# JoernZheng/parallel-data-compression-and-decompression

Hardware: AMD Instinct MI355X
Metric: compress+decompress GB/s (raw bytes / (deflate + inflate time)), .zwz bit-exact (higher is better)
Workload: dtype u8; 1 GPU; 10000 x 262144 B text-like files per GPU -> 50000 chunks of <=65535 B (BASELINE configs[2]); chunk_bytes=65535, max_batch_chunks=51200, parallelism=shard-per-gpu x1

## Files before the change

### parallel-data-compression-and-decompression_amd/csrc/inflate_core.h

```cpp
#pragma once
#include "zwz_common.h"

namespace zwz {

constexpr uint32_t kLitFastBits = 10, kDistFastBits = 8;
constexpr uint32_t kBatch = 64;

enum InflateStatus : uint32_t {
    kInfEnd = 0,
    kInfNeedInput = 1,
    kInfDataError = 2,
    kInfOverflow = 3,
    kInfRunning = 4,
    kInfPending = 5
};

struct InflateTables {
    uint16_t lit_fast[1u << kLitFastBits];
    uint16_t dist_fast[1u << kDistFastBits];
    uint16_t lit_count[16], dist_count[16];
    uint16_t lit_sym[288], dist_sym[32];
    uint16_t lit_walk[2], dist_walk[2];
};

// ... 69 lines not shown
            uint32_t rev = bit_reverse(code, l);
            uint16_t e = (uint16_t)((sorted[idx] << 4) | l);
            for (uint32_t j = rev; j < (1u << fast_bits); j += 1u << l) fast[j] = e;
        }
        code <<= 1;
    }
    return left > 0 ? 1 : 0;
}

constexpr uint32_t kPkLit = 0, kPkMatch = 1, kPkEob = 2, kPkNone = 3, kPkErr = 5, kPkLen = 7;
ZWZ_HD uint16_t pack_lit_entry(uint32_t e ) {
    if (e == 0) return (uint16_t)(kPkNone << 13);
    const uint32_t l = e & 15u, s = e >> 4;
    const uint32_t kind = s < 256u ? kPkLit : s == 256u ? kPkEob : s < 286u ? kPkLen : kPkErr;
    return (uint16_t)(kind << 13 | s << 4 | (l + (kind == kPkLen ? length_extra_bits(s - 257u) : 0u)));
}
ZWZ_HD uint16_t pack_dist_entry(uint32_t e) {
    if (e == 0) return (uint16_t)(kPkNone << 13);
    const uint32_t l = e & 15u, d = e >> 4;
    return (uint16_t)((d < 30u ? kPkMatch : kPkErr) << 13 | d << 5 | (l + (d < 30u ? dist_extra_bits(d) : 0u)));
}
ZWZ_HD uint32_t unpack_lit_entry(uint32_t e) {
    const uint32_t kind = e >> 13, s = (e >> 4) & 511u, skip = e & 15u;
    if (kind == kPkNone) return 0u;
    return s << 4 | (skip - (kind == kPkLen ? length_extra_bits(s - 257u) : 0u));
}
ZWZ_HD uint32_t unpack_dist_entry(uint32_t e) {
    const uint32_t kind = e >> 13, d = (e >> 5) & 31u, skip = e & 31u;
    if (kind == kPkNone) return 0u;
    return d << 4 | (skip - (kind == kPkMatch ? dist_extra_bits(d) : 0u));
}

template <uint32_t kFmt = 0>
ZWZ_HD int decode_symbol(BitReader& br, const uint16_t* fast, uint32_t fast_bits, const uint16_t* count,
                         const uint16_t* sorted) {
    if (br.bits < 15) br.refill();
    uint32_t e = fast[br.peek(fast_bits)];
    if (kFmt == 1u) e = unpack_lit_entry(e); else if (kFmt == 2u) e = unpack_dist_entry(e);
    uint32_t l = e & 15u;
    if (e != 0 && l <= br.bits) { br.drop(l); return (int)(e >> 4); }
    int code = 0, first = 0, index = 0;
    for (uint32_t len = 1; len <= 15; len++) {
        if (br.bits < len) {
            if (len == 1) return -1;
            for (uint32_t l = len; l <= 15; l++) if (count[l]) return -1;
            return -2;
        }
        code |= (int)((br.hold >> (len - 1)) & 1u);
        int c = count[len];
        if (code - c < first) { br.drop(len); return sorted[index + (code - first)]; }
        index += c; first += c; first <<= 1; code <<= 1;
    }
    return -2;
}

struct InflateState {
    BitReader br;
    uint32_t out_pos;
    uint32_t last;
    uint32_t status;
};

ZWZ_HD bool inflate_begin(InflateState& st, const uint8_t* in, uint32_t n, uint32_t ring_mask = 0xffffffffu) {
    st.br.init(in, n, ring_mask); st.out_pos = 0; st.last = 0; st.status = kInfRunning;
    uint32_t cmf, flg;
    if (!st.br.take(8, cmf) || !st.br.take(8, flg)) { st.status = kInfNeedInput; return false; }
    if (((cmf << 8) + flg) % 31u || (cmf & 15u) != 8u || (cmf >> 4) > 7u || (flg & 0x20u)) { st.status = kInfDataError; return false; }
    return true;
}

enum BlockKind : uint32_t { kBlkStored = 0, kBlkHuffman = 1, kBlkStop = 2 };

ZWZ_HD bool inflate_block_type(InflateState& st, uint32_t& type) {
    if (!st.br.take(1, st.last)) { st.status = kInfNeedInput; return false; }
    if (!st.br.take(2, type)) { st.status = kInfNeedInput; return false; }
    return true;
}

ZWZ_HD bool inflate_dyn_begin(InflateState& st, uint8_t* cl , uint32_t& nlen, uint32_t& ndist) {
    BitReader& br = st.br;
    uint32_t ncode, v;
    if (br.bits < 14) br.refill();
    if (br.bits < 14) { st.status = kInfNeedInput; return false; }
    br.take(5, nlen); br.take(5, ndist); br.take(4, ncode);
    nlen += 257; ndist += 1; ncode += 4;
    if (nlen > 286 || ndist > 30) { st.status = kInfDataError; return false; }
    for (uint32_t i = 0; i < 19; i++) cl[i] = 0;
    for (uint32_t i = 0; i < ncode; i++) {
        if (!br.take(3, v)) { st.status = kInfNeedInput; return false; }
        uint32_t o = i < 3 ? 16u + i : i == 3 ? 0u : (i & 1u) ? 8u - ((i - 3u) >> 1) : 8u + ((i - 4u) >> 1);
        cl[o] = (uint8_t)v;
    }
    return true;
}

ZWZ_HD bool inflate_dyn_lengths(InflateState& st, const InflateTables& t, uint8_t* lens, uint32_t nlen, uint32_t ndist) {
    BitReader& br = st.br;
    uint32_t have = 0;
    while (have < nlen + ndist) {
        BitReader save = br;
        int sym = decode_symbol(br, t.dist_fast, 7, t.dist_count, t.dist_sym);
        if (sym == -1) { st.status = kInfNeedInput; return false; }
        if (sym == -2) { st.status = kInfDataError; return false; }
        if (sym < 16) { lens[have++] = (uint8_t)sym; continue; }
        uint32_t prev = 0, rep, xb = sym == 16 ? 2u : sym == 17 ? 3u : 7u, xv;
        if (!br.take(xb, xv)) { br = save; st.status = kInfNeedInput; return false; }
// ... 108 lines not shown
```

### parallel-data-compression-and-decompression_amd/csrc/zwz_kernels.hip

```cpp
#include <hip/hip_runtime.h>

#include <cstdio>
#include <cstdlib>
#include <cstring>
#include <type_traits>

#include "huff_core.h"
#include "inflate_core.h"
#include "stream_core.h"
#include "split_core.h"
#include "lz_core.h"
#include "zwz_md5.h"
#include "zwz_kernels.h"
#include "zwz_device.h"

#ifndef ZWZ_MATCH_EXP
#define ZWZ_MATCH_EXP 0
#endif
#if ZWZ_MATCH_EXP & 16
#define ZWZ_MSTAMP(ph) do { const uint64_t now_ = __builtin_amdgcn_s_memtime(); acc_[(ph)] += (uint32_t)(now_ - stamp_); stamp_ = now_; } while (0)
#else
#define ZWZ_MSTAMP(ph) do { } while (0)
#endif

// ... 1505 lines not shown
        __syncthreads();
    }
    ZWZ_ESTAMP(6);
    if (!in_slots) {
        for (uint32_t i = tid; i < ((n_out + 3) >> 2); i += kThreads) gout[i] = s_out[i];
    } else {
        const uint32_t body = s_blk[0].body_pos, slot_bits = enc_slot_bits<kThreads / 64u, kOutW>(wpw, body, s_blk[0].body_bits), slot0 = (body + 63u) & ~31u;
        const uint32_t sym_end = body + (uint32_t)__builtin_amdgcn_readlane((int)pre_l, kThreads / 64u);
        const uint32_t eob_code = s_blk[0].eob_code, ad_pos = 8u * (s_total_bytes - 4u);
        uint32_t d_of[kThreads / 64u];
#pragma unroll
        for (uint32_t i = 0; i < kThreads / 64u; i++) d_of[i] = body + (uint32_t)__builtin_amdgcn_readlane((int)pre_l, i);
        auto piece = [](uint32_t pos, uint32_t val, uint32_t bit) -> uint32_t {
            const int d = (int)pos - (int)bit;
            return d >= 32 || d <= -32 ? 0u : d >= 0 ? val << d : val >> (-d);
        };
        for (uint32_t j = tid; j < ((n_out + 3) >> 2); j += kThreads) {
            const uint32_t bit = j << 5;
            uint32_t v = j < (slot0 >> 5) ? s_out[j] : 0u;
            v |= piece(sym_end, eob_code, bit);
            if (bit + 32u > ad_pos) v |= piece(ad_pos, adler_be(), bit);
            if (bit + 32u > body && bit < sym_end) {
                uint32_t w = 0;
#pragma unroll
                for (uint32_t i = 1; i < kThreads / 64u; i++) w += d_of[i] <= bit ? 1u : 0u;
                for (; w < kThreads / 64u; w++) {
                    const uint32_t d = body + s_msum[w];
                    if (d >= bit + 32u) break;
                    const int sft = (int)bit - (int)d, len = (int)s_wsum[w];
                    const int lo = sft < 0 ? -sft : 0, hi = len - sft < 32 ? len - sft : 32;
                    if (hi > lo) {
                        const uint32_t at = (uint32_t)((int)(slot0 + w * slot_bits) + sft), aw = at >> 5;
                        const uint32_t x = __builtin_amdgcn_alignbit(s_out[aw + 1u], s_out[aw], at & 31u);
                        const uint32_t mask = (hi >= 32 ? 0xffffffffu : (1u << hi) - 1u) & ~((1u << lo) - 1u);
                        v |= x & mask;
                    }
                }
            }
            gout[j] = v;
        }
    }
    __syncthreads();
    ZWZ_ESTAMP(7);
  }
#if ZWZ_ENC_EXP & 16
    if (tid == ((ZWZ_ENC_EXP & 32) ? 960u : 0u)) for (uint32_t ph = 0; ph < 8; ph++) atomicAdd(&g_enc_times[ph], (unsigned long long)(eacc_[ph] >> 8));
#endif
}

#ifndef ZWZ_INF_EXP
#define ZWZ_INF_EXP 0
#endif
#if ZWZ_INF_EXP & 16
__device__ unsigned long long g_inf_times[8];
#define ZWZ_ISTAMP(ph) do { const uint64_t now_ = __builtin_amdgcn_s_memtime(); iacc_[(ph)] += (uint32_t)(now_ - istamp_); istamp_ = now_; } while (0)
#else
#define ZWZ_ISTAMP(ph) do { } while (0)
#endif
#ifndef ZWZ_INF_WAVES
#define ZWZ_INF_WAVES 5
#endif
constexpr uint32_t kInflateWavesPerSimd = ZWZ_INF_WAVES;
#ifndef ZWZ_WIN_SLOTS
#define ZWZ_WIN_SLOTS 4
#endif
constexpr uint32_t kInfRing = 2048, kInfFill = 1024, kInfMirror = ((8u * ZWZ_WIN_SLOTS + 4u + 15u) / 16u) * 16u;
constexpr uint32_t kWinSlots = ZWZ_WIN_SLOTS;
#ifndef ZWZ_WIN_PARTS
#define ZWZ_WIN_PARTS 2
#endif
constexpr uint32_t kWinParts = ZWZ_WIN_PARTS;

constexpr uint32_t kOwnCap = 1024;

static __device__ __forceinline__ int wave_build_decode_table(const uint8_t* lens, uint32_t n , uint16_t* fast , uint32_t fast_bits,
                                                              uint16_t* count, uint16_t* sorted, uint32_t& max_len, uint16_t* walk0, uint32_t* scr ) {
    const uint32_t lane = lane_id();
    uint32_t* s_cnt = scr; uint32_t* s_pos = scr + 16; uint32_t* s_fc = scr + 32;
    uint32_t l[5];
#pragma unroll
    for (uint32_t r = 0; r < 5; r++) { const uint32_t i = lane + 64u * r; l[r] = i < n ? (uint32_t)lens[i] : 0u; }
    if (lane < 16u) s_cnt[lane] = 0;
    for (uint32_t x = lane; x < (1u << fast_bits) / 8u; x += 64u) reinterpret_cast<uint4*>(fast)[x] = make_uint4(0, 0, 0, 0);
    __builtin_amdgcn_fence(__ATOMIC_ACQ_REL, "wavefront");
#pragma unroll
    for (uint32_t r = 0; r < 5; r++) if (l[r]) atomicAdd(&s_cnt[l[r]], 1u);
    __builtin_amdgcn_fence(__ATOMIC_ACQ_REL, "wavefront");
    int left = 1;
    uint32_t first = 0, index = 0, off = 0, code = 0, my_off = 0, my_fc = 0, my_cnt = 0;
    max_len = 0;
    for (uint32_t len = 1; len < 16u; len++) {
        const uint32_t c = s_cnt[len];
        if (c) max_len = len;
        left = (left << 1) - (int)c;
        if (left < 0) return -1;
        if (len <= fast_bits) { index += c; first += c; first <<= 1; }
        if (lane == len) { my_off = off; my_fc = code; my_cnt = c; }
        off += c; code = (code + c) << 1;
    }
    if (lane < 16u) { s_pos[lane] = my_off; s_fc[lane] = my_fc | my_off << 16; count[lane] = (uint16_t)my_cnt; }
    if (walk0 && lane == 0) { walk0[0] = (uint16_t)first; walk0[1] = (uint16_t)index; }
    __builtin_amdgcn_fence(__ATOMIC_ACQ_REL, "wavefront");
#pragma unroll
    for (uint32_t r = 0; r < 5; r++) {
        if (l[r]) {
            const uint32_t i = lane + 64u * r, pos = atomicAdd(&s_pos[l[r]], 1u);
            sorted[pos] = (uint16_t)i;
            if (l[r] <= fast_bits) {
                const uint32_t w = s_fc[l[r]], cd = (w & 0xffffu) + (pos - (w >> 16));
                const uint16_t e = (uint16_t)((i << 4) | l[r]);
                for (uint32_t j = bit_reverse(cd, l[r]); j < (1u << fast_bits); j += 1u << l[r]) fast[j] = e;
            }
        }
    }
    __builtin_amdgcn_fence(__ATOMIC_ACQ_REL, "wavefront");
    return left > 0 ? 1 : 0;
}

static __device__ __forceinline__ uint32_t wave_dyn_lengths(const uint8_t* ring, uint32_t bp, uint32_t total_bits, const uint16_t* cl_fast ,
                                                            uint8_t* lens, uint32_t want ) {
    const uint32_t lane = lane_id();
    uint32_t have = 0, carry = 0xffffffffu;
    while (have < want) {
        const uint32_t a = bp + lane;
        const uint32_t byte = (a >> 3) & (kInfRing - 1u);
        const uint32_t* w = reinterpret_cast<const uint32_t*>(ring) + (byte >> 2);
        const uint32_t bits = __builtin_amdgcn_alignbyte(w[1], w[0], byte & 3u) >> (a & 7u);
        const uint32_t e = cl_fast[bits & 127u], l = e & 15u, sym = e >> 4;
        const uint32_t xb = sym < 16u ? 0u : sym == 16u ? 2u : sym == 17u ? 3u : 7u, nb = l + xb;
        const uint32_t xv = (bits >> l) & ((1u << xb) - 1u);
        const bool bad = e == 0u || (uint64_t)bp + lane + nb > total_bits;
        const uint32_t jr = lane + (nb ? nb : 1u);
        uint64_t M = 0; uint32_t at = 0;
        while (at < 64u) { M |= 1ull << at; at = (uint32_t)__builtin_amdgcn_readlane((int)jr, (int)at); }
        const bool mine = (M >> lane) & 1ull;
        if (__ballot(mine && bad)) return 0xffffffffu;
        const uint32_t rep = !mine ? 0u : sym < 16u ? 1u : sym == 18u ? 11u + xv : 3u + xv;
        const uint32_t incl = wave_scan_incl(rep), before = have + incl - rep;
        const uint64_t over = __ballot(mine && before + rep > want), in_hdr = __ballot(mine && before < want);
        if (over & in_hdr) return 0xffffffffu;
        const bool live = mine && before < want;
        const uint32_t def = live && sym != 16u ? lane + 1u : 0u;
        const uint32_t near = wave_scan_max_incl(def);
        const uint32_t dval = sym < 16u ? sym : 0u;
        const uint32_t pv = near ? (uint32_t)__shfl((int)dval, (int)(near - 1u)) : carry;
        const uint32_t val = sym == 16u ? pv : dval;
        if (__ballot(live && sym == 16u && pv == 0xffffffffu)) return 0xffffffffu;
        if (live) for (uint32_t k = 0; k < rep; k++) lens[before + k] = (uint8_t)val;
        const uint64_t lv = __ballot(live);
        const uint32_t last = 63u - (uint32_t)__builtin_clzll(lv);
        carry = (uint32_t)__builtin_amdgcn_readlane((int)val, (int)last);
        have = (uint32_t)__builtin_amdgcn_readlane((int)(before + rep), (int)last);
        bp += (uint32_t)__builtin_amdgcn_readlane((int)jr, (int)last);
    }
    return bp;
}

struct InflateWaveMem {
    InflateTables t;
    uint8_t lens[320];
    uint32_t batch[kBatch], pos[kBatch];
    uint32_t sym[kBatch + 1];
    __attribute__((aligned(16))) uint8_t ownb[kOwnCap];
    __attribute__((aligned(16))) uint8_t ring[kInfRing + kInfMirror];
};

template <bool kSerialHeader, bool kStream, uint32_t kSplit = 0>
__global__ __launch_bounds__(kInflateThreads, kInflateWavesPerSimd) void inflate_kernel(const uint8_t* __restrict__ in, const uint64_t* __restrict__ in_off,
                                                                  const uint32_t* __restrict__ in_len, uint32_t n,
                                                                  uint8_t* __restrict__ out, uint64_t out_stride,
                                                                  uint32_t* __restrict__ out_len, uint32_t* __restrict__ status,
                                                                  const uint4* __restrict__ order ,
                                                                  StreamParams sp) {
    __shared__ InflateWaveMem s_mem[kInflateThreads / 64];
    const uint32_t wave = threadIdx.x >> 6, lane = lane_id();
    const uint32_t slot = blockIdx.x * (kInflateThreads / 64) + wave;
    if (slot >= n) return;
    const uint4 oe = order ? order[slot] : make_uint4(0, 0, 0, slot);
    const uint32_t chunk = oe.w;
    InflateWaveMem& m = s_mem[wave];
    const uint8_t* src = in + (order ? ((uint64_t)oe.y << 32 | oe.x) : in_off[chunk]);
    uint8_t* dst;
    uint32_t cap = kChunk;
    uint32_t seg_body = 0, seg_start = 0, seg_base = 0, seg_stream = 0, seg_fin = kSegBad;
    if constexpr (kSplit != 0) {
        static_assert(kStream, "the split forms are stream forms");
        const uint4 sgv = sp.seg[chunk];
        const uint4 sg = make_uint4(__builtin_amdgcn_readfirstlane(sgv.x), __builtin_amdgcn_readfirstlane(sgv.y), __builtin_amdgcn_readfirstlane(sgv.z), __builtin_amdgcn_readfirstlane(sgv.w));
        seg_body = sg.x; seg_stream = sg.y;
        if constexpr (kSplit == 1) { dst = nullptr; cap = kSplitMeasureCap; seg_base = sg.w; }
        else { dst = out + sp.out_off[seg_stream] + (sg.z & ~15u); seg_start = sg.z & 15u; cap = seg_start + sg.w; }
    } else if constexpr (kStream) {
        const uint64_t cap64 = sp.out_cap[chunk];
        if (oe.z >= kStreamMaxIn || cap64 >= kStreamMaxOut) {
            if (lane == 0) { sp.out_len[chunk] = 0; status[chunk] = kStrTooLarge; sp.rec[chunk] = make_uint4(0, 0, 0, kStrTooLarge); }
            return;
        }
        dst = out + sp.out_off[chunk];
        cap = (uint32_t)cap64;
    } else {
        dst = out + (size_t)chunk * out_stride;
    }
    const uint32_t nin = order ? oe.z : in_len[chunk];
    const uint32_t nin16 = (nin + 15u) & ~15u;

    uint32_t fill_end = 0;
    auto top_up = [&](uint32_t pos) {
        pos = __builtin_amdgcn_readfirstlane(pos);
        if (fill_end + kInfRing < pos + kInfFill) fill_end = pos & ~(kInfFill - 1u);
        while (fill_end < pos + kInfFill && fill_end < nin16) {
            const uint32_t o = fill_end + lane * 16u;
            uint4 v = make_uint4(0, 0, 0, 0);
            if (o < nin16) v = *reinterpret_cast<const uint4*>(src + o);
            *reinterpret_cast<uint4*>(m.ring + (o & (kInfRing - 1u))) = v;
            if ((o & (kInfRing - 1u)) < kInfMirror) *reinterpret_cast<uint4*>(m.ring + kInfRing + (o & (kInfRing - 1u))) = v;
            fill_end += kInfFill;
        }
        __builtin_amdgcn_fence(__ATOMIC_ACQ_REL, "wavefront");
    };

    InflateState st;
#if ZWZ_INF_EXP & 16
    uint64_t istamp_ = __builtin_amdgcn_s_memtime();
    uint32_t iacc_[8] = {0, 0, 0, 0, 0, 0, 0, 0};
#endif
    top_up(0);
    uint32_t go = 0;
    uint32_t origin = 0;
    StreamRecord rec{0, 0, 0, kInfRunning};
    if constexpr (kSplit == 2) origin = seg_start;
    auto skip_zeros = [&](uint32_t q) -> uint32_t {
        q = __builtin_amdgcn_readfirstlane(q);
        while (q < nin) {
            const uint32_t base = q & ~15u, o = base + lane * 16u;
            uint32_t hit = 0xffffffffu;
            if (o < nin16) {
                const uint4 v = *reinterpret_cast<const uint4*>(src + o);
                const uint32_t w[4] = {v.x, v.y, v.z, v.w};
#pragma unroll
                for (uint32_t b = 16; b-- > 0;) {
                    const uint32_t at = o + b;
                    if (((w[b >> 2] >> (8u * (b & 3u))) & 255u) && at >= q && at < nin) hit = at;
                }
            }
            const uint64_t any = __ballot(hit != 0xffffffffu);
            if (any) return (uint32_t)__builtin_amdgcn_readlane((int)hit, (int)__builtin_ctzll(any));
            q = base + 64u * 16u;
        }
        return nin;
    };
    if constexpr (kSplit != 0) {
        if (lane == 0) { st.br.init(m.ring, nin, kInfRing - 1u); st.out_pos = seg_start; st.last = 0; st.status = kInfRunning; st.br.seek_bit(seg_body * 8u); }
        go = 1;
    } else if constexpr (kStream) {
        const uint32_t nz = sp.wrap == kWrapGzip ? skip_zeros(0) : nin;
        uint32_t body = 0, sst = kInfRunning;
        if (lane == 0) {
            sst = stream_begin(sp.wrap, src, nin, nz, &body);
            st.br.init(m.ring, nin, kInfRing - 1u); st.out_pos = 0; st.last = 0; st.status = sst;
        }
        body = __builtin_amdgcn_readfirstlane(body);
        go = __builtin_amdgcn_readfirstlane(sst) == kInfRunning;
        if (go) {
            top_up(body);
            if (lane == 0) st.br.seek_bit(body * 8u);
        }
    } else {
        if (lane == 0) go = inflate_begin(st, m.ring, nin, kInfRing - 1u) ? 1u : 0u;
        go = __builtin_amdgcn_readfirstlane(go);
    }
    uint32_t fenced = 0;
    while (go) {
        uint32_t kind = kBlkStop, soff = 0, slen = 0, opos = 0;
        top_up(st.br.bit_pos() >> 3);
        {
            uint32_t v = 0, ok = 0;
            if (lane == 0) { opos = st.out_pos; ok = inflate_block_type(st, v) ? 1u : 0u; }
// ... 37 lines not shown
                }
                if (good) {
                    const int dr = wave_build_decode_table(m.lens + nlen, ndist, m.t.dist_fast, kDistFastBits, m.t.dist_count, m.t.dist_sym, max_len, m.t.dist_walk, m.batch);
                    if (v == 2u) { if (lane == 0) good = inflate_table_ok(st, dr, max_len, false) ? 1u : 0u; good = __builtin_amdgcn_readfirstlane(good); }
                }
                kind = good ? kBlkHuffman : kBlkStop;
            }
        }
        kind = __builtin_amdgcn_readfirstlane(kind);
        if (kind == kBlkStop) break;
        if (kind == kBlkHuffman) {
            __builtin_amdgcn_fence(__ATOMIC_ACQ_REL, "wavefront");
            for (uint32_t x = lane; x < (1u << kLitFastBits); x += 64u) m.t.lit_fast[x] = pack_lit_entry(m.t.lit_fast[x]);
            for (uint32_t x = lane; x < (1u << kDistFastBits); x += 64u) m.t.dist_fast[x] = pack_dist_entry(m.t.dist_fast[x]);
            __builtin_amdgcn_fence(__ATOMIC_ACQ_REL, "wavefront");
        }
        if (kind == kBlkStored) {
            soff = __builtin_amdgcn_readfirstlane(soff); slen = __builtin_amdgcn_readfirstlane(slen);
            opos = __builtin_amdgcn_readfirstlane(opos);
            uint32_t room = cap - opos, cp = slen < room ? slen : room;
            if constexpr (kSplit != 1) {
                const uint32_t head = min(cp, (16u - (opos & 15u)) & 15u);
                if (lane < head) dst[opos + lane] = src[soff + lane];
                const uint32_t s0 = soff + head, d0 = opos + head, sh = s0 & 3u;
                const uint32_t* sw = reinterpret_cast<const uint32_t*>(src + (s0 & ~3u));
                uint32_t nvec = (cp - head) >> 4;
                while (nvec && (s0 & ~3u) + 16u * nvec + 4u > nin16) nvec--;
                for (uint32_t v = lane; v < nvec; v += 64) {
                    const uint32_t* q = sw + 4u * v;
                    const uint32_t w0 = q[0], w1 = q[1], w2 = q[2], w3 = q[3], w4 = q[4];
                    *reinterpret_cast<uint4*>(dst + d0 + 16u * v) = make_uint4(__builtin_amdgcn_alignbyte(w1, w0, sh), __builtin_amdgcn_alignbyte(w2, w1, sh),
                                                                                __builtin_amdgcn_alignbyte(w3, w2, sh), __builtin_amdgcn_alignbyte(w4, w3, sh));
                }
                for (uint32_t i = head + 16u * nvec + lane; i < cp; i += 64) dst[opos + i] = src[soff + i];
            }
            uint32_t stop = 0;
            if (lane == 0) {
                st.out_pos += cp;
                if (cp < slen) st.status = kInfOverflow;
                stop = st.status != kInfRunning;
            }
            if (__builtin_amdgcn_readfirstlane(stop)) break;
        } else {
            enum : uint32_t { kLit = 0, kMatch = 1, kEob = 2, kSlow = 3, kNeed = 4, kErr = 5 };
            static_assert(kLit == kPkLit && kMatch == kPkMatch && kEob == kPkEob && kSlow == kPkNone && kErr == kPkErr, "the packed entries carry this enum");
            uint32_t bp = 0, opos_u = 0;
            if (lane == 0) { bp = st.br.bit_pos(); opos_u = st.out_pos; }
            bp = __builtin_amdgcn_readfirstlane(bp); opos_u = __builtin_amdgcn_readfirstlane(opos_u);
            const uint32_t total_bits = nin * 8u;
            uint32_t block_done = 0, stop_status = kInfRunning;
            ZWZ_ISTAMP(0);
            while (!block_done) {
                top_up(bp >> 3);
                uint32_t nsym = 0;
                uint32_t at = 0;
                constexpr uint32_t kOrbitEnd = 0xffffu;
#pragma unroll 1
              for (uint32_t wb = 0; wb < 64u * kWinSlots * kWinParts; wb += 64u * kWinSlots) {
                uint32_t inf[kWinSlots];
                const uint32_t near_end_s = __builtin_amdgcn_readfirstlane((uint32_t)((uint64_t)bp + wb + 64u * kWinSlots + 64u > total_bits));
                const uint32_t a0 = bp + wb + lane;
                const uint32_t byte0 = (a0 >> 3) & (kInfRing - 1u);
                uint32_t wd[2u * kWinSlots + 1u];
                {
                    const uint32_t* w = reinterpret_cast<const uint32_t*>(m.ring) + (byte0 >> 2);
#pragma unroll
                    for (uint32_t i = 0; i < 2u * kWinSlots + 1u; i++) wd[i] = w[i];
                }
#pragma unroll
                for (uint32_t r = 0; r < kWinSlots; r++) {
                    const uint32_t lo = __builtin_amdgcn_alignbyte(wd[2u * r + 1u], wd[2u * r], byte0), hi = __builtin_amdgcn_alignbyte(wd[2u * r + 2u], wd[2u * r + 1u], byte0);
                    const uint64_t bits = (((uint64_t)hi << 32) | lo) >> (a0 & 7u);
                    const uint32_t e = m.t.lit_fast[(uint32_t)bits & ((1u << kLitFastBits) - 1u)];
                    const uint32_t skip = e & 15u;
                    const uint32_t de = m.t.dist_fast[(uint32_t)(bits >> skip) & ((1u << kDistFastBits) - 1u)];
                    const bool is_len = (e >> 13) == kPkLen;
                    uint32_t kind = is_len ? de >> 13 : e >> 13;
                    const uint32_t nb = skip + (is_len ? de & 31u : 0u);
                    if (near_end_s) {
                        const int32_t avail = (int32_t)total_bits - (int32_t)(a0 + r * 64u);
                        if (avail <= 0 || ((kind <= kEob || kind == kErr) && (int32_t)nb > avail)) kind = kNeed;
                    }
                    inf[r] = kind | (nb << 3);
                }
                ZWZ_ISTAMP(1);
                uint32_t jr[kWinSlots];
#pragma unroll
                for (uint32_t r = 0; r < kWinSlots; r++) {
                    const uint32_t nbits = inf[r] >> 3;
                    jr[r] = (((inf[r] & 7u) <= kMatch) & (nbits != 0u)) ? wb + r * 64u + lane + nbits : kOrbitEnd;
                }
                uint64_t M[kWinSlots];
#pragma unroll
                for (uint32_t r = 0; r < kWinSlots; r++) {
                    uint64_t mk = 0;
                    const uint32_t lim = wb + 64u * (r + 1u);
                    auto hop = [&] { asm volatile("s_bitset1_b64 %0, %1" : "+s"(mk) : "s"(at)); at = (uint32_t)__builtin_amdgcn_readlane((int)jr[r], (int)at); };
                    while (at < lim) {
                        hop();
                        if (at >= lim) break;
                        hop();
                        if (at >= lim) break;
                        hop();
                        if (at >= lim) break;
                        hop();
                    }
                    M[r] = mk;
                }
#pragma unroll
                for (uint32_t r = 0; r < kWinSlots; r++) {
                    const uint32_t rank = nsym + rank_in(M[r]);
                    if (((M[r] >> lane) & 1ull) && rank <= kBatch) m.sym[rank] = (wb + r * 64u + lane) | inf[r] << 10;
                    nsym += (uint32_t)__popcll(M[r]);
                }
                ZWZ_ISTAMP(2);
                if (at >= kOrbitEnd || nsym > kBatch) break;
              }
                __builtin_amdgcn_fence(__ATOMIC_ACQ_REL, "wavefront");
                uint32_t cur = 0, k = 0, stop = 0xffu, opos_new = opos_u;
                {
                    const uint32_t have = (uint32_t)(lane < nsym);
                    const uint32_t sy = m.sym[lane];
                    const uint32_t kd = (sy >> 10) & 7u, s_off = sy & 0x3ffu, s_nb = sy >> 13;
                    uint32_t v;
                    {
                        const uint32_t a = bp + s_off;
                        const uint32_t byte = (a >> 3) & (kInfRing - 1u);
                        const uint32_t* w = reinterpret_cast<const uint32_t*>(m.ring) + (byte >> 2);
                        const uint32_t lo = __builtin_amdgcn_alignbyte(w[1], w[0], byte & 3u), hi = __builtin_amdgcn_alignbyte(w[2], w[1], byte & 3u);
                        const uint64_t bits = (((uint64_t)hi << 32) | lo) >> (a & 7u);
                        const uint32_t e = m.t.lit_fast[(uint32_t)bits & ((1u << kLitFastBits) - 1u)];
                        const uint32_t s = (e >> 4) & 511u, skip = e & 15u;
                        const uint32_t c = (s - 257u) & 31u;
                        const uint32_t xb = length_extra_bits(c);
                        const uint32_t len = length_base(c) + 3u + ((uint32_t)(bits >> ((skip - xb) & 15u)) & ((1u << xb) - 1u));
                        const uint64_t rest = bits >> skip;
                        const uint32_t de = m.t.dist_fast[(uint32_t)rest & ((1u << kDistFastBits) - 1u)];
                        const uint32_t d = (de >> 5) & 31u, dxb = dist_extra_bits(d) & 15u;
                        const uint32_t dist = dist_base(d) + 1u + ((uint32_t)(rest >> (((de & 31u) - dxb) & 31u)) & ((1u << dxb) - 1u));
                        v = kd == kMatch ? (len << 16) | dist : kd == kLit ? s : 0u;
                    }
                    const uint32_t is_lit = have & (uint32_t)(kd == kLit), is_match = have & (uint32_t)(kd == kMatch), mlen = v >> 16;
                    const uint32_t ol = is_lit + is_match * mlen;
                    const uint32_t sc = wave_scan_incl(ol);
                    const uint32_t pos = opos_u + sc - ol;
                    uint32_t ends;
                    if constexpr (kStream)
                        ends = have & ((uint32_t)(kd >= kEob) | (is_lit & (uint32_t)(pos >= cap)) |
                                       (is_match & ((uint32_t)((v & 0xffffu) > pos - origin) | (uint32_t)(mlen > cap - pos))));
                    else
                        ends = have & ((uint32_t)(kd >= kEob) | (is_lit & (uint32_t)(pos >= kChunk)) |
                                       (is_match & ((uint32_t)((v & 0xffffu) > pos) | (uint32_t)(pos + mlen > kChunk))));
                    const uint64_t C = __ballot(ends != 0);
                    if (C) {
                        const uint32_t lc = (uint32_t)__builtin_ctzll(C);
                        const uint32_t c_kind = (uint32_t)__builtin_amdgcn_readlane((int)kd, (int)lc), c_val = (uint32_t)__builtin_amdgcn_readlane((int)v, (int)lc);
                        const uint32_t c_off = (uint32_t)__builtin_amdgcn_readlane((int)s_off, (int)lc), c_nb = (uint32_t)__builtin_amdgcn_readlane((int)s_nb, (int)lc);
                        opos_new = (uint32_t)__builtin_amdgcn_readlane((int)pos, (int)lc);
                        cur = c_off;
                        k = lc;
                        if (c_kind == kLit) { stop = kErr; stop_status = kInfOverflow; }
                        else if (c_kind == kMatch) { stop = kErr; stop_status = (c_val & 0xffffu) > opos_new - origin ? kInfDataError : kInfOverflow; }
                        else if (c_kind == kEob) { cur += c_nb; stop = kEob; }
                        else { stop = c_kind; if (c_kind == kNeed) stop_status = kInfNeedInput; else if (c_kind == kErr) stop_status = kInfDataError; }
                    } else if (nsym > kBatch) {
                        k = kBatch;
                        cur = m.sym[kBatch] & 0x3ffu;
                        opos_new = opos_u + (uint32_t)__builtin_amdgcn_readlane((int)sc, 63);
                    } else {
                        k = nsym;
                        cur = (uint32_t)__builtin_amdgcn_readlane((int)(s_off + s_nb), (int)(nsym - 1u));
                        opos_new = opos_u + (uint32_t)__builtin_amdgcn_readlane((int)sc, 63);
                    }
                    m.batch[lane] = v;
                    m.pos[lane] = lane < k ? pos : 0xffffffffu;
                }
                bp += cur;
                __builtin_amdgcn_fence(__ATOMIC_ACQ_REL, "wavefront");
                ZWZ_ISTAMP(3);
                const uint32_t bstart = opos_u;
                const uint32_t bbytes = opos_new - bstart;
                opos_u = opos_new;
                if constexpr (kSplit != 1) {
                const bool mapped = bbytes <= kOwnCap;
                if (mapped) {
                    for (uint32_t i = lane; i < (bbytes + 15u) >> 4; i += 64u) reinterpret_cast<uint4*>(m.ownb)[i] = make_uint4(0, 0, 0, 0);
                    __builtin_amdgcn_fence(__ATOMIC_ACQ_REL, "wavefront");
                    if (lane < k) m.ownb[m.pos[lane] - bstart] = (uint8_t)(lane + 1u);
                    __builtin_amdgcn_fence(__ATOMIC_ACQ_REL, "wavefront");
                    uint32_t carry = 0;
                    for (uint32_t j0 = 0; j0 < bbytes; j0 += 64) {
                        const uint32_t o = max(wave_scan_max_incl((uint32_t)m.ownb[j0 + lane]), carry);
                        m.ownb[j0 + lane] = (uint8_t)o;
                        carry = (uint32_t)__builtin_amdgcn_readlane((int)o, 63);
                    }
                    __builtin_amdgcn_fence(__ATOMIC_ACQ_REL, "wavefront");
                }
                ZWZ_ISTAMP(4);
                auto owner = [&](uint32_t pos, uint32_t& ov, uint32_t& op) {
                    uint32_t lo = 0;
                    if (mapped) lo = (uint32_t)m.ownb[pos - bstart] - 1u;
                    else {
#pragma unroll
                        for (uint32_t stp = 32; stp >= 1; stp >>= 1) { const uint32_t q = m.pos[(lo + stp) & 63u]; if (q <= pos) lo += stp; }
                    }
                    ov = m.batch[lo]; op = m.pos[lo];
                };
                auto source_of = [&](uint32_t at, uint32_t op, uint32_t d, bool live) -> uint32_t {
                    const uint32_t off = at - op;
                    uint32_t from = at - d;
                    if (__ballot(live && off >= d)) from = off < d ? from : op - d + off % (d | (uint32_t)!live);
                    return from;
                };
                bool need_fence = false;
                for (uint32_t j0 = 0; j0 < bbytes; j0 += 64) {
                    const uint32_t pos = bstart + j0 + lane;
                    const bool in = j0 + lane < bbytes;
                    uint32_t ov = 0, op = 0;
                    owner(in ? pos : bstart, ov, op);
                    bool lit = ov < 256u;
                    uint32_t src = source_of(pos, op, ov & 0xffffu, in && !lit);
                    while (__ballot(in && !lit && src >= bstart)) {
                        const bool go2 = in && !lit && src >= bstart;
                        uint32_t ov2 = 0, op2 = 0;
                        owner(go2 ? src : bstart, ov2, op2);
                        const uint32_t s2 = source_of(src, op2, ov2 & 0xffffu, go2 && ov2 >= 256u);
                        if (go2) {
                            if (ov2 < 256u) { lit = true; ov = ov2; }
                            else src = s2;
                        }
                    }
                    const uint64_t far = __ballot(in && !lit && src + 1u > fenced);
                    if (far && !(ZWZ_INF_EXP & 2)) { __builtin_amdgcn_fence(__ATOMIC_ACQ_REL, "workgroup"); __builtin_amdgcn_s_waitcnt(0); fenced = bstart; }
                    if (in) dst[pos] = lit ? (uint8_t)ov : __hip_atomic_load(&dst[src], __ATOMIC_RELAXED, __HIP_MEMORY_SCOPE_AGENT);
                    (void)need_fence;
                }
                }
                ZWZ_ISTAMP(5);
                if (stop == kEob) block_done = 1;
                else if (stop == kSlow) {
                    uint32_t k1 = 0, d1 = 0, nbp = bp, nop = opos_u, stt = kInfRunning;
                    if (lane == 0) {
                        st.br.seek_bit(bp); st.out_pos = opos_u;
                        bool d;
                        if constexpr (kStream) k1 = inflate_decode_batch<true, true>(st, m.t, cap, m.batch, m.pos, d, 1u, origin);
                        else k1 = inflate_decode_batch<true>(st, m.t, kChunk, m.batch, m.pos, d, 1u);
                        d1 = d; nbp = st.br.bit_pos(); nop = st.out_pos; stt = st.status;
                    }
                    k1 = __builtin_amdgcn_readfirstlane(k1); d1 = __builtin_amdgcn_readfirstlane(d1);
                    bp = __builtin_amdgcn_readfirstlane(nbp); opos_u = __builtin_amdgcn_readfirstlane(nop);
                    stt = __builtin_amdgcn_readfirstlane(stt);
                    __builtin_amdgcn_fence(__ATOMIC_ACQ_REL, "wavefront");
                    if constexpr (kSplit != 1) if (k1) {
                        const uint32_t mv = m.batch[0], mp = m.pos[0];
                        if (mv < 256u) { if (lane == 0) dst[mp] = (uint8_t)mv; }
                        else {
                            const uint32_t len = mv >> 16, dist = mv & 0xffffu;
                            const uint32_t from = mp - dist, span = len < dist ? len : dist;
                            if (from + span > fenced) {
                                __builtin_amdgcn_fence(__ATOMIC_ACQ_REL, "workgroup");
                                __builtin_amdgcn_s_waitcnt(0);
                                fenced = mp;
                            }
                            for (uint32_t i = lane; i < len; i += 64) dst[mp + i] = __hip_atomic_load(&dst[from + (i % dist)], __ATOMIC_RELAXED, __HIP_MEMORY_SCOPE_AGENT);
                        }
                    }
                    if (d1) { block_done = 1; stop_status = stt; }
                } else if (stop != 0xffu) { block_done = 1; }
            }
            uint32_t halt = 0;
            if (lane == 0) {
                st.out_pos = opos_u;
                if (stop_status != kInfRunning) st.status = stop_status;
                else st.br.seek_bit(bp);
                halt = st.status != kInfRunning;
            }
            if (__builtin_amdgcn_readfirstlane(halt)) break;
        }
        if constexpr (kSplit != 0) {
            uint32_t fin = kSegBad;
            if (lane == 0) fin = split_stop(st.last, kind == kBlkStored && slen == 0u);
            seg_fin = __builtin_amdgcn_readfirstlane(fin);
            if (seg_fin != kSegBad) break;
        } else if constexpr (kStream) {
            uint32_t more = 0, next = 0;
            if (lane == 0 && st.last) {
                const uint32_t q = (st.br.bit_pos() + 7u) >> 3;
                st.status = stream_trailer(sp.wrap, src, nin, q, st.out_pos, st.out_pos - origin, rec, &next);
                more = st.status == kInfRunning;
                if (!more) rec.status = st.status;
            }
            if (__builtin_amdgcn_readfirstlane(more)) {
                const uint32_t nz = skip_zeros(next);
                uint32_t body = 0, sst = kInfRunning;
                if (lane == 0) { sst = gzip_next_member(src, nin, nz, &body); st.status = sst; st.last = 0; }
                body = __builtin_amdgcn_readfirstlane(body);
                if (__builtin_amdgcn_readfirstlane(sst) != kInfRunning) break;
                origin = __builtin_amdgcn_readfirstlane(st.out_pos);
                top_up(body);
                if (lane == 0) st.br.seek_bit(body * 8u);
                continue;
            }
            if (__builtin_amdgcn_readfirstlane((uint32_t)(st.status != kInfRunning))) break;
        } else {
            uint32_t fin = 0;
            if (lane == 0 && st.last) { st.status = kInfEnd; fin = 1; }
            if (__builtin_amdgcn_readfirstlane(fin)) break;
        }
    }
    if constexpr (kSplit == 1) {
        if (lane == 0) sp.meas[chunk] = make_uint4(seg_fin, seg_base + ((st.br.bit_pos() + 7u) >> 3), st.out_pos, st.status);
    } else if constexpr (kSplit == 2) {
        if (lane == 0 && !(seg_fin != kSegBad && st.out_pos == cap)) sp.bad[seg_stream] = 1;
    } else if constexpr (kStream) {
        if (lane == 0) {
            sp.out_len[chunk] = st.out_pos; status[chunk] = st.status;
            sp.rec[chunk] = make_uint4(rec.checked, rec.expect, rec.has_check, st.status);
        }
    } else {
        if (lane == 0) { out_len[chunk] = st.out_pos; status[chunk] = st.status; }
    }
#if ZWZ_INF_EXP & 16
    ZWZ_ISTAMP(6);
    if (lane == 0) for (uint32_t ph = 0; ph < 8; ph++) atomicAdd(&g_inf_times[ph], (unsigned long long)(iacc_[ph] >> 8));
#endif
}

#define ZWZ_TRY(x) do { hipError_t e_ = (x); if (e_ != hipSuccess) return e_; } while (0)

constexpr uint32_t kProbeRounds = 384;
__global__ __launch_bounds__(kLinksThreads) void exchange_order_probe_kernel(uint32_t* __restrict__ violations) {
    extern __shared__ __attribute__((aligned(16))) uint32_t tab[];
    constexpr uint32_t kBuckets = 32768u;
    uint32_t* area = tab + kBuckets + 4u;
    const uint32_t tid = threadIdx.x, lane = lane_id(), wave = tid >> 6;
    for (uint32_t i = tid; i < kBuckets; i += kLinksThreads) tab[i] = 0xdead0000u + i;
    for (uint32_t i = tid; i < 4096u; i += kLinksThreads) area[i] = i;
    __syncthreads();
    if (wave != 0) {
        uint4* a4 = reinterpret_cast<uint4*>(area) + (wave - 1u) * 128u + lane;
        uint4 v = a4[0];
        for (uint32_t it = 0; it < 3u * kProbeRounds; it++) {
            a4[64 * (it & 1u)] = make_uint4(v.x + it, v.y ^ it, v.z + lane, v.w);
            v = a4[64 * ((it + 1u) & 1u)];
        }
        if (v.x == 0xffffffffu && v.y == 0x12345678u) violations[1] = v.z;
        return;
    }
    typedef __attribute__((address_space(3))) uint32_t* lds_word_ptr;
    const uint32_t tab_a = (uint32_t)(uintptr_t)(lds_word_ptr)tab;
    uint32_t bad = 0, rng = 0x9e3779b9u * (lane + 1u) + 0x85ebca6bu * (blockIdx.x + 1u);
    for (uint32_t r = 0; r < kProbeRounds; r++) {
        rng = rng * 1664525u + 1013904223u;
        const uint32_t spread = 1u << (3u * (r % 6u));
        const uint32_t base = (0x9e3779b1u * (r + 17u * blockIdx.x)) & (kBuckets - 1u) & ~(spread - 1u);
        const uint32_t a = base + ((rng >> 11) & (spread - 1u));
        const uint32_t la = tab_a + 4u * a, mine = 0x10000u * (r + 1u) + lane;
        uint32_t pre, old, post;
        asm volatile("ds_read_b32 %0, %3\n\ts_waitcnt lgkmcnt(0)\n\t"
                     "ds_wrxchg_rtn_b32 %1, %3, %4\n\ts_waitcnt lgkmcnt(0)\n\t"
                     "ds_read_b32 %2, %3\n\ts_waitcnt lgkmcnt(0)"
                     : "=&v"(pre), "=&v"(old), "=&v"(post) : "v"(la), "v"(mine) : "memory");
        uint32_t want = pre, last = lane;
        for (uint32_t j = 0; j < 64; j++) {
            const uint32_t aj = (uint32_t)__builtin_amdgcn_readlane((int)a, (int)j);
            if (aj != a) continue;
            if (j < lane) want = 0x10000u * (r + 1u) + j;
            if (j > lane) last = j;
        }
        bad += (uint32_t)(old != want) + (uint32_t)(post != 0x10000u * (r + 1u) + last);
    }
    if (bad) atomicAdd(violations, bad);
}

hipError_t probe_exchange_order(hipStream_t s, bool* holds) {
    uint32_t* d = nullptr;
    uint32_t h[2] = {1, 0};
// ... 212 lines not shown
    };
    auto grouped_add = [&](uint32_t c, bool live) -> uint32_t {
        uint32_t slot = 0;
        uint64_t todo = __builtin_amdgcn_ballot_w64(live);
        if (todo) {
            const uint32_t c0 = (uint32_t)__builtin_amdgcn_readlane((int)c, (int)__builtin_ctzll(todo));
            const uint64_t m = __builtin_amdgcn_ballot_w64(live && c == c0);
            if (__popcll(todo & ~m) > 8) {
                if (live) slot = atomicAdd(&s_bin[c], 1u);
                return slot;
            }
        }
        while (todo) {
            const uint32_t c0 = (uint32_t)__builtin_amdgcn_readlane((int)c, (int)__builtin_ctzll(todo));
            const uint64_t m = __builtin_amdgcn_ballot_w64(live && c == c0);
            uint32_t base = 0;
            if (lane_id() == (uint32_t)__builtin_ctzll(m)) base = atomicAdd(&s_bin[c0], (uint32_t)__popcll(m));
            base = (uint32_t)__builtin_amdgcn_readlane((int)base, (int)__builtin_ctzll(m));
            if (live && c == c0) slot = base + rank_in(m);
            todo &= ~m;
        }
        return slot;
    };
    for (uint32_t i = tid; i - tid < n; i += 1024u) (void)grouped_add(i < n ? cls(in_len(i)) : 0u, i < n);
    __syncthreads();
    const bool keep = __syncthreads_count(tid < 256u && s_bin[tid] != 0u) <= 2;
    if (keep) {
        for (uint32_t i = tid; i < n; i += 1024u) { const uint64_t off = in_off[i]; order[i] = make_uint4((uint32_t)off, (uint32_t)(off >> 32), in_len(i), i); }
        return;
    }
    if (tid < 64u) {
        const uint32_t a = s_bin[4 * tid], b = s_bin[4 * tid + 1], c = s_bin[4 * tid + 2], d = s_bin[4 * tid + 3];
        const uint32_t own = a + b + c + d, ex = wave_scan_incl(own) - own;
        s_bin[4 * tid] = ex; s_bin[4 * tid + 1] = ex + a; s_bin[4 * tid + 2] = ex + a + b; s_bin[4 * tid + 3] = ex + a + b + c;
    }
    __syncthreads();
    for (uint32_t i = tid; i - tid < n; i += 1024u) {
        const uint32_t len = i < n ? in_len(i) : 0u;
        const uint32_t slot = grouped_add(cls(len), i < n);
        if (i < n) { const uint64_t off = in_off[i]; order[slot] = make_uint4((uint32_t)off, (uint32_t)(off >> 32), len, i); }
    }
}

hipError_t launch_inflate(const InflateArgs& a, hipStream_t s) {
    if (a.n == 0) return hipSuccess;
    const uint32_t per = kInflateThreads / 64;
    if (a.order) hipLaunchKernelGGL(inflate_order_kernel<uint32_t>, dim3(1), dim3(1024), 0, s, a.in_off, a.in_len, a.n, a.order);
    if (a.serial_header) hipLaunchKernelGGL((inflate_kernel<true, false>), dim3((a.n + per - 1) / per), dim3(kInflateThreads), 0, s, a.in, a.in_off, a.in_len, a.n, a.out,
                                            a.out_stride, a.out_len, a.status, (const uint4*)a.order, StreamParams{});
    else hipLaunchKernelGGL((inflate_kernel<false, false>), dim3((a.n + per - 1) / per), dim3(kInflateThreads), 0, s, a.in, a.in_off, a.in_len, a.n, a.out,
                            a.out_stride, a.out_len, a.status, (const uint4*)a.order, StreamParams{});
#if ZWZ_INF_EXP & 16
    if (getenv("ZWZ_INF_TIMES")) {
        unsigned long long h[8], z[8] = {0};
        ZWZ_TRY(hipStreamSynchronize(s));
        ZWZ_TRY(hipMemcpyFromSymbol(h, HIP_SYMBOL(g_inf_times), sizeof h));
        ZWZ_TRY(hipMemcpyToSymbol(HIP_SYMBOL(g_inf_times), z, sizeof z));
        fprintf(stderr, "ZWZ_INF_TIMES n=%u header=%llu decode=%llu orbit=%llu symbols=%llu owners=%llu copy=%llu other=%llu\n", a.n, h[0], h[1], h[2], h[3], h[4], h[5], h[6]);
    }
#endif
    return hipGetLastError();
}

hipError_t launch_inflate_streams(const InflateStreamArgs& a, hipStream_t s) {
    if (a.n == 0) return hipSuccess;
    const uint32_t per = kInflateThreads / 64;
    hipLaunchKernelGGL(inflate_order_kernel<uint64_t>, dim3(1), dim3(1024), 0, s, a.in_off, a.in_len, a.n, a.order);
    const StreamParams sp{a.out_off, a.out_cap, a.out_len, a.rec, a.wrap};
    if (a.serial_header) hipLaunchKernelGGL((inflate_kernel<true, true>), dim3((a.n + per - 1) / per), dim3(kInflateThreads), 0, s, a.in, a.in_off, nullptr, a.n, a.out,
                                            0, nullptr, a.status, (const uint4*)a.order, sp);
    else hipLaunchKernelGGL((inflate_kernel<false, true>), dim3((a.n + per - 1) / per), dim3(kInflateThreads), 0, s, a.in, a.in_off, nullptr, a.n, a.out,
                            0, nullptr, a.status, (const uint4*)a.order, sp);
    return hipGetLastError();
}

hipError_t launch_inflate_split(const InflateSplitArgs& a, hipStream_t s) {
    if (a.n == 0) return hipSuccess;
    const uint32_t per = kInflateThreads / 64;
    hipLaunchKernelGGL(inflate_order_kernel<uint64_t>, dim3(1), dim3(1024), 0, s, a.seg_in_off, a.seg_in_len, a.n, a.order);
    StreamParams sp{};
    sp.out_off = a.out_off; sp.seg = a.seg; sp.meas = a.meas; sp.bad = a.bad;
    const dim3 grid((a.n + per - 1) / per), block(kInflateThreads);
#define ZWZ_SPLIT_LAUNCH(h, k) hipLaunchKernelGGL((inflate_kernel<h, true, k>), grid, block, 0, s, a.in, a.seg_in_off, nullptr, a.n, a.out, 0, nullptr, nullptr, (const uint4*)a.order, sp)
    if (a.measure) { if (a.serial_header) ZWZ_SPLIT_LAUNCH(true, 1); else ZWZ_SPLIT_LAUNCH(false, 1); }
    else { if (a.serial_header) ZWZ_SPLIT_LAUNCH(true, 2); else ZWZ_SPLIT_LAUNCH(false, 2); }
#undef ZWZ_SPLIT_LAUNCH
    return hipGetLastError();
}

}
```

Baseline: 22.12 GB/s.

## Resolve long Huffman codes in-wave instead of falling back to serial decode

When the orbit walk of the parallel inflate stops on a symbol whose code is longer than the fast table covers, the wave now decodes that long literal/length/distance cooperatively. Each lane probes one code length using canonical-code prefix scans. The decoded value is stored in a small side buffer, the symbol's entry is patched, and the orbit walk continues. This avoids dropping into the lane-0 sequential decode path and ending the batch early. It adds ballot/scan work per long code, a cap of eight such symbols per round, and extra registers and shared memory. Counters for rounds, sequential fallbacks and resolved symbols are added to the instrumentation.

```diff
diff --git a/parallel-data-compression-and-decompression_amd/csrc/inflate_core.h b/parallel-data-compression-and-decompression_amd/csrc/inflate_core.h
--- a/parallel-data-compression-and-decompression_amd/csrc/inflate_core.h
+++ b/parallel-data-compression-and-decompression_amd/csrc/inflate_core.h
@@ -145,6 +145,43 @@
         index += c; first += c; first <<= 1; code <<= 1;
     }
     return -2;
+}
+
+ZWZ_HD bool long_code_probe(uint32_t x, uint32_t l , uint32_t count_l, uint32_t before, uint32_t weight_before, uint32_t& idx) {
+    const uint32_t first = weight_before >> (15u - l);
+    const uint32_t d = bit_reverse(x & ((1u << l) - 1u), l) - first;
+    idx = before + d;
+    return d < count_l;
+}
+struct LongSymbol { uint32_t kind, nb, value; };
+template <class Pick>
+ZWZ_HD LongSymbol long_symbol(uint64_t bits, const InflateTables& t, Pick pick) {
+    const LongSymbol none{kPkNone, 0u, 0u};
+    const uint32_t e = t.lit_fast[(uint32_t)bits & ((1u << kLitFastBits) - 1u)];
+    uint32_t s = (e >> 4) & 511u, skip = e & 15u;
+    if ((e >> 13) == kPkNone) {
+        const uint32_t p = pick(t.lit_count, (uint32_t)bits & 0x7fffu);
+        if (!p) return none;
+        s = t.lit_sym[p >> 4];
+        if (s < 256u) return LongSymbol{kPkLit, p & 15u, s};
+        if (s == 256u || s >= 286u) return none;
+        skip = (p & 15u) + length_extra_bits(s - 257u);
+    } else if ((e >> 13) != kPkLen) return none;
+    const bool long_len = (e >> 13) == kPkNone;
+    const uint32_t c = s - 257u, xb = length_extra_bits(c);
+    const uint32_t len = c == 28u ? 258u : length_base(c) + 3u + ((uint32_t)(bits >> (skip - xb)) & ((1u << xb) - 1u));
+    const uint64_t rest = bits >> skip;
+    const uint32_t de = t.dist_fast[(uint32_t)rest & ((1u << kDistFastBits) - 1u)];
+    uint32_t d = (de >> 5) & 31u, dl = (de & 31u) - dist_extra_bits(d);
+    if ((de >> 13) == kPkNone) {
+        const uint32_t p = pick(t.dist_count, (uint32_t)rest & 0x7fffu);
+        if (!p) return none;
+        d = t.dist_sym[p >> 4]; dl = p & 15u;
+        if (d >= 30u) return none;
+    } else if ((de >> 13) != kPkMatch || !long_len) return none;
+    const uint32_t dxb = dist_extra_bits(d);
+    const uint32_t dist = dist_base(d) + 1u + ((uint32_t)(rest >> dl) & ((1u << dxb) - 1u));
+    return LongSymbol{kPkMatch, skip + dl + dxb, len << 16 | dist};
 }
 
 struct InflateState {
diff --git a/parallel-data-compression-and-decompression_amd/csrc/zwz_kernels.hip b/parallel-data-compression-and-decompression_amd/csrc/zwz_kernels.hip
--- a/parallel-data-compression-and-decompression_amd/csrc/zwz_kernels.hip
+++ b/parallel-data-compression-and-decompression_amd/csrc/zwz_kernels.hip
@@ -1581,10 +1581,12 @@
 #define ZWZ_INF_EXP 0
 #endif
 #if ZWZ_INF_EXP & 16
-__device__ unsigned long long g_inf_times[8];
+__device__ unsigned long long g_inf_times[8], g_inf_counts[4];
+#define ZWZ_ICOUNT(c) do { icnt_[(c)]++; } while (0)
 #define ZWZ_ISTAMP(ph) do { const uint64_t now_ = __builtin_amdgcn_s_memtime(); iacc_[(ph)] += (uint32_t)(now_ - istamp_); istamp_ = now_; } while (0)
 #else
 #define ZWZ_ISTAMP(ph) do { } while (0)
+#define ZWZ_ICOUNT(c) do { } while (0)
 #endif
 #ifndef ZWZ_INF_WAVES
 #define ZWZ_INF_WAVES 5
@@ -1600,6 +1602,7 @@
 #endif
 constexpr uint32_t kWinParts = ZWZ_WIN_PARTS;
 
+constexpr uint32_t kLongCap = 8;
 constexpr uint32_t kOwnCap = 1024;
 
 static __device__ __forceinline__ int wave_build_decode_table(const uint8_t* lens, uint32_t n , uint16_t* fast , uint32_t fast_bits,
@@ -1690,6 +1693,7 @@
     uint8_t lens[320];
     uint32_t batch[kBatch], pos[kBatch];
     uint32_t sym[kBatch + 1];
+    uint32_t side[kLongCap];
     __attribute__((aligned(16))) uint8_t ownb[kOwnCap];
     __attribute__((aligned(16))) uint8_t ring[kInfRing + kInfMirror];
 };
@@ -1751,7 +1755,7 @@
     InflateState st;
 #if ZWZ_INF_EXP & 16
     uint64_t istamp_ = __builtin_amdgcn_s_memtime();
-    uint32_t iacc_[8] = {0, 0, 0, 0, 0, 0, 0, 0};
+    uint32_t iacc_[8] = {0, 0, 0, 0, 0, 0, 0, 0}, icnt_[3] = {0, 0, 0};
 #endif
     top_up(0);
     uint32_t go = 0;
@@ -1895,7 +1899,9 @@
             ZWZ_ISTAMP(0);
             while (!block_done) {
                 top_up(bp >> 3);
+                ZWZ_ICOUNT(0);
                 uint32_t nsym = 0;
+                uint32_t nlong = 0;
                 uint32_t at = 0;
                 constexpr uint32_t kOrbitEnd = 0xffffu;
 #pragma unroll 1
@@ -1935,8 +1941,11 @@
                 }
                 uint64_t M[kWinSlots];
 #pragma unroll
+                for (uint32_t r = 0; r < kWinSlots; r++) M[r] = 0;
+              for (;;) {
+#pragma unroll
                 for (uint32_t r = 0; r < kWinSlots; r++) {
-                    uint64_t mk = 0;
+                    uint64_t mk = M[r];
                     const uint32_t lim = wb + 64u * (r + 1u);
                     auto hop = [&] { asm volatile("s_bitset1_b64 %0, %1" : "+s"(mk) : "s"(at)); at = (uint32_t)__builtin_amdgcn_readlane((int)jr[r], (int)at); };
                     while (at < lim) {
@@ -1950,6 +1959,35 @@
                     }
                     M[r] = mk;
                 }
+                if (__builtin_expect(at != kOrbitEnd || near_end_s || nlong >= kLongCap || (ZWZ_INF_EXP & 4), 1)) break;
+                uint32_t rs = 0, last = 0, li = kErr;
+#pragma unroll
+                for (uint32_t r = 0; r < kWinSlots; r++)
+                    if (M[r]) { rs = r; last = 63u - (uint32_t)__builtin_clzll(M[r]); li = (uint32_t)__builtin_amdgcn_readlane((int)inf[r], (int)last); }
+                if (__builtin_expect((li & 7u) != kSlow, 1)) break;
+                const uint32_t loff = wb + rs * 64u + last, a = bp + loff;
+                const uint32_t byte = (a >> 3) & (kInfRing - 1u);
+                const uint32_t* w = reinterpret_cast<const uint32_t*>(m.ring) + (byte >> 2);
+                const uint32_t lo = __builtin_amdgcn_alignbyte(w[1], w[0], byte & 3u), hi = __builtin_amdgcn_alignbyte(w[2], w[1], byte & 3u);
+                const LongSymbol ls = long_symbol((((uint64_t)hi << 32) | lo) >> (a & 7u), m.t, [&](const uint16_t* count, uint32_t x) -> uint32_t {
+                    const uint32_t l = lane & 15u, c = count[l], wt = c << (15u - l);
+                    uint32_t idx = 0;
+                    const bool hit = long_code_probe(x, l | (uint32_t)(l == 0u), c, wave_scan_incl(c) - c, wave_scan_incl(wt) - wt, idx) && lane - 1u < 15u;
+                    const uint64_t b = __ballot(hit);
+                    if (!b) return 0u;
+                    const uint32_t won = (uint32_t)__builtin_ctzll(b);
+                    return won | (uint32_t)__builtin_amdgcn_readlane((int)idx, (int)won) << 4;
+                });
+                if (__builtin_amdgcn_readfirstlane(ls.kind) == kPkNone) break;
+                const uint32_t l_nb = __builtin_amdgcn_readfirstlane(ls.nb);
+                const uint32_t patched = __builtin_amdgcn_readfirstlane(ls.kind) | l_nb << 3 | (nlong + 1u) << 9;
+#pragma unroll
+                for (uint32_t r = 0; r < kWinSlots; r++) if (rs == r && lane == last) inf[r] = patched;
+                if (lane == 0) m.side[nlong] = ls.value;
+                nlong++;
+                ZWZ_ICOUNT(2);
+                at = loff + l_nb;
+              }
 #pragma unroll
                 for (uint32_t r = 0; r < kWinSlots; r++) {
                     const uint32_t rank = nsym + rank_in(M[r]);
@@ -1964,7 +2002,7 @@
                 {
                     const uint32_t have = (uint32_t)(lane < nsym);
                     const uint32_t sy = m.sym[lane];
-                    const uint32_t kd = (sy >> 10) & 7u, s_off = sy & 0x3ffu, s_nb = sy >> 13;
+                    const uint32_t kd = (sy >> 10) & 7u, s_off = sy & 0x3ffu, s_nb = (sy >> 13) & 63u;
                     uint32_t v;
                     {
                         const uint32_t a = bp + s_off;
@@ -1983,6 +2021,7 @@
                         const uint32_t dist = dist_base(d) + 1u + ((uint32_t)(rest >> (((de & 31u) - dxb) & 31u)) & ((1u << dxb) - 1u));
                         v = kd == kMatch ? (len << 16) | dist : kd == kLit ? s : 0u;
                     }
+                    if (nlong) { const uint32_t sx = sy >> 19; if (have & (uint32_t)(sx != 0u)) v = m.side[(sx - 1u) & (kLongCap - 1u)]; }
                     const uint32_t is_lit = have & (uint32_t)(kd == kLit), is_match = have & (uint32_t)(kd == kMatch), mlen = v >> 16;
                     const uint32_t ol = is_lit + is_match * mlen;
                     const uint32_t sc = wave_scan_incl(ol);
@@ -2083,6 +2122,7 @@
                 if (stop == kEob) block_done = 1;
                 else if (stop == kSlow) {
                     uint32_t k1 = 0, d1 = 0, nbp = bp, nop = opos_u, stt = kInfRunning;
+                    ZWZ_ICOUNT(1);
                     if (lane == 0) {
                         st.br.seek_bit(bp); st.out_pos = opos_u;
                         bool d;
@@ -2166,6 +2206,7 @@
 #if ZWZ_INF_EXP & 16
     ZWZ_ISTAMP(6);
     if (lane == 0) for (uint32_t ph = 0; ph < 8; ph++) atomicAdd(&g_inf_times[ph], (unsigned long long)(iacc_[ph] >> 8));
+    if (lane == 0) for (uint32_t c = 0; c < 3; c++) atomicAdd(&g_inf_counts[c], (unsigned long long)icnt_[c]);
 #endif
 }
 
@@ -2484,11 +2525,13 @@
                             a.out_stride, a.out_len, a.status, (const uint4*)a.order, StreamParams{});
 #if ZWZ_INF_EXP & 16
     if (getenv("ZWZ_INF_TIMES")) {
-        unsigned long long h[8], z[8] = {0};
+        unsigned long long h[8], c[4], z[8] = {0};
         ZWZ_TRY(hipStreamSynchronize(s));
         ZWZ_TRY(hipMemcpyFromSymbol(h, HIP_SYMBOL(g_inf_times), sizeof h));
+        ZWZ_TRY(hipMemcpyFromSymbol(c, HIP_SYMBOL(g_inf_counts), sizeof c));
         ZWZ_TRY(hipMemcpyToSymbol(HIP_SYMBOL(g_inf_times), z, sizeof z));
-        fprintf(stderr, "ZWZ_INF_TIMES n=%u header=%llu decode=%llu orbit=%llu symbols=%llu owners=%llu copy=%llu other=%llu\n", a.n, h[0], h[1], h[2], h[3], h[4], h[5], h[6]);
+        ZWZ_TRY(hipMemcpyToSymbol(HIP_SYMBOL(g_inf_counts), z, sizeof c));
+        fprintf(stderr, "ZWZ_INF_TIMES n=%u header=%llu decode=%llu orbit=%llu symbols=%llu owners=%llu copy=%llu other=%llu rounds=%llu sequential=%llu resolved=%llu\n", a.n, h[0], h[1], h[2], h[3], h[4], h[5], h[6], c[0], c[1], c[2]);
     }
 #endif
     return hipGetLastError();
```

After: 22.31 GB/s (median of 6 runs). Within noise of the previous version (+0.9%).
